# Gavinli-lgf/belief-planning

Hardware: AMD Instinct MI355X
Metric: branch-MPC solves/sec (whole node), highway N=20 M=3 branches, batch 4096 egos (higher is better)
Workload: dtype f64; 1 GPU; highway BranchMPC_CVaR closed loop, N=20, NB=1, m=3 (T=64, U=61), 4096 egos per GPU; batch_per_gpu=4096, global_batch=4096, world_size=1, parallelism=ego-sharded dp1, loop=per step: k_env + solve launches

## Files before the change

### __graft_entry__.py

```python
import os
import sys

REPO = os.path.dirname(os.path.abspath(__file__))
PKG = os.path.join(REPO, "belief-planning_amd")
for _p in (REPO, PKG, os.path.join(REPO, "tests")):
    if _p not in sys.path:
        sys.path.insert(0, _p)


def build() -> None:
    from bmpc import _lib
    _lib.build(force=True, verbose=True)
    _lib.load()
    import hostsim_lib
    hostsim_lib.build()
    import bmpc.plan
    import MPC_branch
    import highway_branch_dyn
    print("build ok:", _lib.SO_PATH)


def smoke() -> None:
    import numpy as np
    from bmpc import plan
    from bmpc.scenarios import highway_desc, highway_policy_rows, seeded_batch
    from oracle.ecos_ipm import ecos_solve
    from oracle.model import HighwayModel, highway_policies
    from oracle.tree import CVaRController

    B = 4
    x, z, xref, tgt = seeded_batch(B, seed=0)
    pl = plan.BatchPlan(highway_desc(N=10, NB=1), B)
    pl.set_policies(highway_policy_rows(tgt))
    r = pl.solve(x, z, xref)
    assert np.all(r["status"] >= 0), r["status"]
    mdl = HighwayModel(10, 0.1, highway_policies(0.1, tgt[0]))
    Fx = np.array([[0., 1, 0, 0], [0, -1, 0, 0], [0, 0, 0, 1], [0, 0, 0, -1]])
    c = CVaRController(mdl, 10, 1, np.diag([0., 3, 3, 10]), np.diag([1., 100]), Fx,
                       [4 * 3.6 - 1.25, -1.25, .25, .25], np.kron(np.eye(2), [1, -1]).T,
                       [6., 6., .3, .3], [0, 300], xref[0], 0.9, solver=ecos_solve)
    c.solve(x[0], z[0], xref[0])
    J_ref = c.last_info["x"][-1]
    assert abs(r["J"][0] - J_ref) <= 1e-6 * max(1.0, abs(J_ref)), (r["J"][0], J_ref)
    assert np.max(np.abs(r["upred"][0, 0] - c.uPred[0])) <= 1e-4
    import scipy.sparse as sp
    from oracle.qp_ipm import osqp_like_solve
# ... 18 lines not shown
```

### belief-planning_amd/bmpc/_lib.py

```python
from __future__ import annotations

import ctypes as C
import os
import subprocess

PKG_DIR = os.path.dirname(os.path.dirname(os.path.abspath(__file__)))
REPO = os.path.dirname(PKG_DIR)
CSRC = os.path.join(PKG_DIR, "csrc")
INCLUDE = os.path.join(REPO, "include")
SO_PATH = os.path.join(PKG_DIR, "libbmpc.so")
PROF_SO_PATH = os.path.join(PKG_DIR, "libbmpc_prof.so")
HIPCC = os.environ.get("HIPCC", "/opt/rocm/bin/hipcc")
EXTRA_FLAGS = []
ARCH = os.environ.get("BMPC_OFFLOAD_ARCH", "gfx950")


class BmpcUnavailable(RuntimeError):
    """libbmpc.so (the MI355X kernels) cannot be loaded or has no usable HIP device."""


EXPERIMENTAL = os.path.join(CSRC, "experimental")


def _phased() -> bool:
# ... 21 lines not shown

def build(force: bool = False, verbose: bool = False, profile: bool = False) -> str:
    out = PROF_SO_PATH if profile else SO_PATH
    stamp = out + ".srchash"
    want = source_hash()
    if not force and os.path.exists(out) and os.path.exists(stamp):
        with open(stamp) as f:
            if f.read().strip() == want:
                return out
    import tempfile
    from concurrent.futures import ThreadPoolExecutor
    flags = [f"--offload-arch={ARCH}", "-O3", "-std=c++17", "-fPIC",
             "-Wno-unused-value", "-Wno-unused-result", "-Wno-pass-failed",
             *(["-DBMPC_PROFILE"] if profile else []), *EXTRA_FLAGS, "-I" + INCLUDE, "-I" + CSRC,
             *(["-I" + EXPERIMENTAL] if _phased() else [])]
    with tempfile.TemporaryDirectory(prefix="bmpc_build_") as tmp:
        objs = [os.path.join(tmp, os.path.basename(src) + ".o") for src in sources()]
        cmds = [[HIPCC, *flags, "-c", src, "-o", obj] for src, obj in zip(sources(), objs)]
        if verbose:
            for c in cmds:
                print(" ".join(c))
        jobs = int(os.environ.get("MAX_JOBS", "0")) or min(len(cmds), os.cpu_count() or 1)
        with ThreadPoolExecutor(jobs) as pool:
            for f in [pool.submit(subprocess.check_call, c) for c in cmds]:
                f.result()
        link = [HIPCC, f"--offload-arch={ARCH}", "-shared", "-fPIC", *objs, "-o", out + ".tmp"]
        if verbose:
            print(" ".join(link))
        subprocess.check_call(link)
    os.replace(out + ".tmp", out)
    with open(stamp, "w") as f:
        f.write(want + "\n")
    return out


_LIB = None

_SIGS = {
    "bmpc_last_error": (C.c_char_p, []),
    "bmpc_abi_version": (C.c_int, []),
    "bmpc_open": (C.c_int, [C.c_int, C.c_void_p]),
    "bmpc_close": (C.c_int, [C.c_void_p]),
    "bmpc_plan_create": (C.c_int, [C.c_void_p, C.c_void_p, C.c_int, C.c_void_p]),
    "bmpc_plan_destroy": (C.c_int, [C.c_void_p]),
    "bmpc_plan_info": (C.c_int, [C.c_void_p, C.c_void_p]),
    "bmpc_set_policies": (C.c_int, [C.c_void_p, C.c_void_p, C.c_void_p]),
    "bmpc_reset": (C.c_int, [C.c_void_p, C.c_void_p]),
    "bmpc_get_policies": (C.c_int, [C.c_void_p, C.c_void_p]),
    "bmpc_solve": (C.c_int, [C.c_void_p] + [C.c_void_p] * 9),
    "bmpc_solve_device": (C.c_int, [C.c_void_p] + [C.c_void_p] * 10),
    "bmpc_get_tree": (C.c_int, [C.c_void_p] + [C.c_void_p] * 6),
    "bmpc_get_warm_start": (C.c_int, [C.c_void_p] * 4),
    "bmpc_get_counters": (C.c_int, [C.c_void_p] * 2),
    "bmpc_set_warm_start": (C.c_int, [C.c_void_p] * 5),
    "bmpc_get_robust_warm_start": (C.c_int, [C.c_void_p] * 4),
    "bmpc_set_robust_warm_start": (C.c_int, [C.c_void_p] * 5),
    "bmpc_set_transform": (C.c_int, [C.c_void_p] * 5),
    "bmpc_set_fx": (C.c_int, [C.c_void_p] * 3),
    "bmpc_get_transform": (C.c_int, [C.c_void_p] * 4),
    "bmpc_get_branch_dp": (C.c_int, [C.c_void_p] * 2),
    "bmpc_enable_timing": (C.c_int, [C.c_void_p, C.c_int]),
    "bmpc_timing": (C.c_int, [C.c_void_p, C.c_void_p, C.c_void_p]),
    "bmpc_model_eval": (C.c_int, [C.c_void_p, C.c_void_p, C.c_void_p, C.c_int] + [C.c_void_p] * 12),
    "bmpc_model_eval_ref": (C.c_int, [C.c_void_p, C.c_void_p, C.c_void_p, C.c_int, C.c_void_p, C.c_void_p, C.c_int]
                            + [C.c_void_p] * 12),
    "bmpc_set_lane_ref": (C.c_int, [C.c_void_p, C.c_int, C.c_void_p, C.c_void_p]),
# ... 84 lines not shown
```

### belief-planning_amd/csrc/bmpc_core.h

```cpp
#pragma once

#include <stddef.h>
#include <stdint.h>

#include "bmpc.h"

#ifndef BMPC_PHASE_NOCSR
#define BMPC_PHASE_NOCSR 1
#endif
#if BMPC_PHASE_NOCSR && defined(__HIP_DEVICE_COMPILE__)
#define BMPC_FN_CALLS __attribute__((not_tail_called))
#else
#define BMPC_FN_CALLS
#endif
#if defined(__HIPCC__)
#include <hip/hip_runtime.h>
#define BMPC_HD __host__ __device__ __forceinline__
#if defined(BMPC_INLINE_ALL)
#define BMPC_FN __host__ __device__ __forceinline__
#else
#define BMPC_FN __host__ __device__ __attribute__((noinline)) BMPC_FN_CALLS
#endif
#else
#define BMPC_HD inline
#define BMPC_FN inline
#endif

#include <math.h>

namespace bmpc {

#if defined(__HIP_DEVICE_COMPILE__)
#if defined(BMPC_FLAT_SLAB)
#define BMPC_AS_GLOBAL
#else
#define BMPC_AS_GLOBAL __attribute__((address_space(1)))
#endif
#define BMPC_AS_LDS __attribute__((address_space(3)))
#define BMPC_AS_CONST __attribute__((address_space(4)))
#else
#define BMPC_AS_GLOBAL
#define BMPC_AS_LDS
#define BMPC_AS_CONST
#endif
typedef BMPC_AS_GLOBAL double gdouble;
typedef BMPC_AS_LDS double ldouble;
typedef const BMPC_AS_GLOBAL int32_t gint;
// ... 17 lines not shown
#define BMPC_TOPO_COUNT_(n) +1
enum { BMPC_TOPO_N = 0 BMPC_TOPO_FIELDS(BMPC_TOPO_COUNT_) };
#define BMPC_TOPO_MEMBER_(n) IP n;
template <class IP>
struct TopoT {
  BMPC_TOPO_FIELDS(BMPC_TOPO_MEMBER_)
};
typedef const BMPC_AS_LDS int32_t lint;
typedef TopoT<gint*> Topo;
typedef TopoT<lint*> TopoL;

enum { XF_S = 0, XF_BX = BMPC_MAX_N * BMPC_MAX_N, XF_SON = XF_BX + BMPC_MAX_FX, XF_BXSET = XF_SON + 1,
       XF_FX = XF_BXSET + 1, XF_FXSET = XF_FX + BMPC_MAX_FX * BMPC_MAX_N, XF_ROWS = XF_FXSET + 1,
       XF_BROWS = XF_ROWS + BMPC_MAX_FX * BMPC_MAX_N, XF_ROWSET = XF_BROWS + BMPC_MAX_FX,
       XF_COUNT = XF_ROWSET + 1 };

enum { ECO_FX = 0, ECO_W1 = BMPC_MAX_FX * BMPC_MAX_N, ECO_QQ = ECO_W1 + BMPC_MAX_N * BMPC_MAX_N,
       ECO_BX = ECO_QQ + BMPC_MAX_N * BMPC_MAX_N, ECO_COUNT = ECO_BX + BMPC_MAX_FX };

struct Plan {
  bmpc_plan_desc desc;
  int n, d, N, NB, m, nFx, nFu, Nc;
  int Ncol, zNB;
  int T, U, nbranch, bdim, ncones, nlevels;
  int oX, oU, oRho, oSig, oMup, oMum, oS, oJ, nv;
  int neq;
  int rFx, rFu, rRisk, rPos, nlp, nrows;
  int ng;
  int nsm;
  int lds_M, lds_piv, lds_rhs, lds_rhs2, lds_red, nlds;
  int lds_w, lds_wu, lds_fx, lds_fu, nconst;
  int nlds_lean;
  int lds_scr, nscr;
  int cgrp;
  int maxq;
  double W1[BMPC_MAX_N * BMPC_MAX_N];
  double Wu[BMPC_MAX_D * BMPC_MAX_D];
  double QQ[BMPC_MAX_N * BMPC_MAX_N];
  double RR[BMPC_MAX_D * BMPC_MAX_D];
  Topo t;
  int toff[BMPC_TOPO_N];
  int ntab;
  const double* lref;
  int nlref;
};

template <class X>
BMPC_HD double fxv(const BMPC_AS_CONST Plan& P, const X& ex, int r, int j) {
  if constexpr (X::kTransform) return ex.eco[ECO_FX + r * P.n + j];
  else return ex.lds[P.lds_fx + r * P.n + j];
}
template <class X>
BMPC_HD double fuv(const BMPC_AS_CONST Plan& P, const X& ex, int r, int j) {
  return ex.lds[P.lds_fu + r * P.d + j];
}
template <class X>
BMPC_HD double w1v(const BMPC_AS_CONST Plan& P, const X& ex, int r, int j) {
  if constexpr (X::kTransform) return ex.eco[ECO_W1 + r * P.n + j];
  else return P.W1[r * P.n + j];
}
template <class X>
BMPC_HD double qqv(const BMPC_AS_CONST Plan& P, const X& ex, int i, int j) {
  if constexpr (X::kTransform) return ex.eco[ECO_QQ + i * P.n + j];
  else return P.QQ[i * P.n + j];
}
template <class X>
// ... 324 lines not shown
```

### belief-planning_amd/csrc/bmpc_dev.h

```cpp
#pragma once

#include <hip/hip_runtime.h>

#include <type_traits>

#include "bmpc_env_merge.h"
#include "bmpc_env_quad.h"
#include "bmpc_hmm.h"
#include "bmpc_plan.h"
#include "bmpc_qp.h"
#include "bmpc_qpplan.h"
#include "bmpc_record.h"
#include "bmpc_solve.h"

namespace bmpc {
namespace dev {

#ifndef BMPC_WPE
#define BMPC_WPE 4
#endif


#ifndef BMPC_DPP_REDUCE
#define BMPC_DPP_REDUCE 1
// ... 2 lines not shown
constexpr bool kDppBlock = BMPC_DPP_REDUCE == 1 || BMPC_DPP_REDUCE == 2;

template <bool TR, bool TL = true>
struct DevExecT {
  static constexpr bool kTransform = TR;
  static constexpr bool kCoupLds = TL;
  using tab_ptr = typename std::conditional<TL, lint*, gint*>::type;
  int lane;
  ldouble* lds;
  tab_ptr tab;
  ldouble* eco;
  static constexpr int nlanes = 64;
  static constexpr bool kBqpWave = true;
  static constexpr bool kInlineG = true;
  static constexpr bool kRowLanes = true;
  __device__ double rlane(double v, int l) const {
    return __hiloint2double(__builtin_amdgcn_readlane(__double2hiint(v), l),
                            __builtin_amdgcn_readlane(__double2loint(v), l));
  }
  static constexpr int kTaskLanes = 4;
  static constexpr int kConeRegRows = 8;
  __device__ double tsum(double v) const {
    v += dpp_d<0xB1>(v);
    v += dpp_d<0x4E>(v);
    return v;
  }
  template <int S>
  __device__ double tget(double v) const { return dpp_d<S | (S << 2) | (S << 4) | (S << 6)>(v); }
  __device__ double gsum(double v, int g) const { return group_reduce<0, kDppWave>(v, g); }
  __device__ double gmax(double v, int g) const { return group_reduce<1, kDppWave>(v, g); }
  __device__ double gmin(double v, int g) const { return group_reduce<2, kDppWave>(v, g); }
  __device__ void sync() const { __syncthreads(); }
  __device__ bool uniform(bool b) const { return __builtin_amdgcn_readfirstlane((int)b) != 0; }
  __device__ double sum(double v) const { return wave_reduce<0, kDppWave>(v); }
  __device__ double max(double v) const { return wave_reduce<1, kDppWave>(v); }
  __device__ double min(double v) const { return wave_reduce<2, kDppWave>(v); }
  template <int K>
  __device__ void sum_n(double* v) const {
#pragma unroll
    for (int k = 0; k < K; ++k) v[k] = sum(v[k]);
  }
  template <int K>
  __device__ void min_n(double* v) const {
#pragma unroll
    for (int k = 0; k < K; ++k) v[k] = min(v[k]);
  }
};

using DevExec = DevExecT<false>;

#ifndef BMPC_BLK_RED2
#define BMPC_BLK_RED2 1
#endif
template <bool TR, bool TL, int NW>
struct DevBlockExecT {
  static constexpr bool kTransform = TR;
  static constexpr bool kCoupLds = TL;
  using tab_ptr = typename std::conditional<TL, lint*, gint*>::type;
  int lane;
  ldouble* lds;
  tab_ptr tab;
  ldouble* eco;
  ldouble* red;
  static constexpr int nlanes = 64 * NW;
  static constexpr int kBatchDiv = NW;
  static constexpr bool kRowLanes = true;
  static constexpr int kTaskLanes = 4;
  static constexpr int kConeRegRows = NW == 4 ? 4 : 8;
  static constexpr int kConeBatch = NW == 4 ? 2 : 4;
  static constexpr int kRedMax = 16;
  __device__ double tsum(double v) const {
    v += dpp_d<0xB1>(v);
    v += dpp_d<0x4E>(v);
    return v;
  }
  template <int S>
  __device__ double tget(double v) const { return dpp_d<S | (S << 2) | (S << 4) | (S << 6)>(v); }
  __device__ double gsum(double v, int g) const { return group_reduce<0, kDppBlock>(v, g); }
  __device__ double gmax(double v, int g) const { return group_reduce<1, kDppBlock>(v, g); }
  __device__ double gmin(double v, int g) const { return group_reduce<2, kDppBlock>(v, g); }
  __device__ void sync() const { __syncthreads(); }
  __device__ bool uniform(bool b) const { return __builtin_amdgcn_readfirstlane((int)b) != 0; }
  template <int OP, int K>
  __device__ void reduce(double* v) const {
    static_assert(K <= kRedMax, "reduction scratch");
#pragma unroll
    for (int k = 0; k < K; ++k) v[k] = wave_reduce<OP, kDppBlock>(v[k]);
    const int wv = lane >> 6;
#if BMPC_BLK_RED2
    ldouble* turn = red + 2 * kRedMax * NW + wv;
    const int odd = __builtin_amdgcn_readfirstlane((int)*turn);
    ldouble* buf = red + (odd ? kRedMax * NW : 0);
    if ((lane & 63) == 0) {
#pragma unroll
      for (int k = 0; k < K; ++k) buf[k * NW + wv] = v[k];
      *turn = odd ? 0.0 : 1.0;
    }
#else
    ldouble* buf = red;
    __syncthreads();
    if ((lane & 63) == 0)
#pragma unroll
      for (int k = 0; k < K; ++k) red[k * NW + wv] = v[k];
// ... 515 lines not shown
```

### belief-planning_amd/csrc/bmpc_ipm.h

```cpp
#pragma once

#include <type_traits>

#include "bmpc_tree.h"
#include "bmpc_wave.h"

#ifndef BMPC_EQUIL
#define BMPC_EQUIL 1
#endif
#ifndef BMPC_EQUIL_ITERS
#define BMPC_EQUIL_ITERS 3
#endif
#ifndef BMPC_TS_POST_RB_MIN
#define BMPC_TS_POST_RB_MIN 8
#endif
#ifndef BMPC_TS_POST_RB
#define BMPC_TS_POST_RB 4
#endif
#ifndef BMPC_PAIR_REFINE
#define BMPC_PAIR_REFINE 1
#endif
#ifndef BMPC_BLK_WAVE_SUBST
#define BMPC_BLK_WAVE_SUBST 1
#endif
// ... 3455 lines not shown
            const int b = t.cone_b[k], ii = t.cone_i[k];
            on = col == P.oSig + b || col == P.oMup + b + ii || col == P.oMum + b + ii ||
                 (t.br_child0[c] >= 0 && col == P.oRho + c);
          } else {
            on = col == P.oJ || col == P.oRho;
          }
          if (on) m = fmax(m, 1.0 / (ge[t.cone_off[k]] * cf));
        }
        if (col < P.oMup) {
          const int b = col < P.oSig ? col - P.oRho : col - P.oSig;
          m = fmax(m, 1.0 / (ae[T * NX + b] * cf));
        } else if (col >= P.oMum && col < P.oS) {
          const int j = col - P.oMum;
          m = fmax(m, fabs(p[j] / P.desc.ralpha) / (ae[T * NX + j / P.m] * cf));
        }
      }
      cm[col] = m;
    }
    ex.sync();
    auto fac = [](double v) { return fabs(v) < 1e-6 ? 1.0 : sqrt(v); };
    for (int i = ex.lane; i < nv; i += ex.nlanes) xe[i] *= fac(cm[i]);
    for (int i = ex.lane; i < neq; i += ex.nlanes) ae[i] *= fac(am[i]);
    for (int i = ex.lane; i < nr; i += ex.nlanes) ge[i] *= fac(gm[i]);
    ex.sync();
  }
}

struct IpmResult {
  int exit_flag;
  int iters;
  double pcost;
};

template <class X, int NX, int NU>
BMPC_HD IpmResult ipm_solve(const X ex, const Ctx& C) {
  CPlan& P = *C.P;
  CLayout& L = *C.L;
  gdouble* ws = C.ws;
  const int nv = P.nv, neq = P.neq, nr = P.nrows;
  gdouble* x = ws + L.x;
  gdouble* y = ws + L.y;
  gdouble* z = ws + L.z;
  gdouble* s = ws + L.s;
  gdouble* lam = ws + L.lam;
  gdouble* x1 = ws + L.x1;
  gdouble* y1 = ws + L.y1;
  gdouble* z1 = ws + L.z1;
  gdouble* x2 = ws + L.x2;
  gdouble* y2 = ws + L.y2;
  gdouble* z2 = ws + L.z2;
  gdouble* dz = ws + L.dz;
  gdouble* ds = ws + L.ds;
  gdouble* rx = ws + L.rx;
  gdouble* ry = ws + L.ry;
  gdouble* rz = ws + L.rz;
  gdouble* hv = ws + L.hvec;
  gdouble* bv = ws + L.bvec;
  gdouble* tA = ws + L.ta;
  gdouble* tA2 = ws + L.ta2;
  gdouble* ya = ws + L.ya;
  gdouble* ra = ws + L.ra;
  gdouble* rb = ws + L.rb;
  gdouble* rc = ws + L.rc;
  const double feastol = P.desc.feastol, abstol = P.desc.abstol, reltol = P.desc.reltol;
  const double deg = (double)(P.nlp + P.ncones);
  IpmResult res{EXIT_MAXIT, 0, 0.0};
  BMPC_PROF(ws, L, PROF_TOTAL);
  BMPC_TIC(t_init);
// ... 262 lines not shown
#else
        lane_batch<8>(ex, 0, nv, [&](int i) { return x[i] + (alpha * x2[i]); }, [&](int i, double v) { x[i] = v; });
        lane_batch(ex, 0, neq, [&](int i) { return y[i] + (alpha * y2[i]); }, [&](int i, double v) { y[i] = v; });
#endif
        struct ZS { double z, s; };
        lane_batch<4>(ex, 0, nr, [&](int i) { return ZS{z[i] + alpha * z2[i], s[i] + alpha * rc[i]}; },
                   [&](int i, ZS v) { z[i] = v.z; s[i] = v.s; });
        tau += alpha * dtau;
        kap += alpha * dkap;
        ex.sync();
      }
    }
    if (!ok) {
      BMPC_TRACE("   backtrack (it %d) to the best iterate (it %d, score %.3e)\n", it, best_it, best_score);
      if (best_score < 1e300 && (ws[L.misc + MISC_BEST] != best_score || ws[L.misc + MISC_BEST + 1] != best_tau)) {
        res.exit_flag = EXIT_GUARD;
        res.iters = it;
        return res;
      }
      const bool inacc = bs_ok_cx && bs_pres < 1e-4 && bs_dres < 1e-4 &&
                         (bs_gap < 5e-5 || (bs_relgap >= 0.0 && bs_relgap < 5e-5));
      lane_batch<16>(ex, 0, nv, [&](int i) { return ws[L.bestx + i] / best_tau; }, [&](int i, double v) { ws[L.sol + i] = v; });
      ex.sync();
      res.exit_flag = inacc ? EXIT_OPTIMAL + EXIT_INACC : EXIT_NUMERICS;
      res.iters = it;
      res.pcost = bs_pcost;
      (void)best_it;
      return res;
    }
  }
  return res;
}

}
```

### belief-planning_amd/csrc/bmpc_plan.cpp

```cpp
#include <stdlib.h>
#include "bmpc_plan.h"

#include <algorithm>

#include <math.h>
#include <string.h>

#include <deque>

namespace bmpc {

namespace {

void sqrtm_sym(const double* A, int n, double* out) {
  double a[BMPC_MAX_N][BMPC_MAX_N], v[BMPC_MAX_N][BMPC_MAX_N];
  for (int i = 0; i < n; ++i)
    for (int j = 0; j < n; ++j) {
      a[i][j] = A[i * n + j];
      v[i][j] = i == j ? 1.0 : 0.0;
    }
  for (int sweep = 0; sweep < 100; ++sweep) {
    double off = 0.0;
    for (int i = 0; i < n; ++i)
      for (int j = i + 1; j < n; ++j) off += a[i][j] * a[i][j];
// ... 245 lines not shown
  hp.cone_c.push_back(-1);
  hp.cone_q.push_back(2 + d);
  hp.cone_off.push_back(row);
  hp.u_cone[0] = k;
  row += 2 + d;
  P.nrows = row;
  P.maxq = 0;
  for (int q : hp.cone_q) P.maxq = q > P.maxq ? q : P.maxq;
  while (P.cgrp < 64 && P.maxq > 8 * P.cgrp) P.cgrp <<= 1;
  if (desc.controller != BMPC_CTRL_CVAR) {
    P.oS = T * n + U * d;
    P.oRho = P.oSig = P.oMup = P.oMum = P.oS;
    P.oJ = P.oS + T * P.Nc;
    P.ncones = 0;
    P.nv = P.oJ;
    P.neq = T * n;
    P.rFx = 0;
    P.rFu = T * P.Nc;
    P.rRisk = P.rFu + U * P.nFu;
    P.rPos = P.rRisk;
    P.nlp = P.rPos + T * P.Nc;
    P.nrows = P.nlp;
    P.ng = 0;
    P.nsm = 0;
  }
  const int ncoup = P.nsm * P.nsm + 3 * P.nsm;
  P.lds_red = 0;
  P.lds_w = 0;
  P.lds_wu = P.lds_w + n * n;
  P.lds_fx = P.lds_wu + d * d;
  P.lds_fu = P.lds_fx + P.nFx * n;
  P.nconst = P.lds_fu + P.nFu * d;
  P.lds_scr = std::max(64, (P.nconst + 7) & ~7);
  P.nscr = desc.controller == BMPC_CTRL_CVAR && P.lds_scr + ncoup + T * P.Nc <= 1248 ? T * P.Nc : 0;
  P.lds_piv = P.lds_scr + P.nscr;
  P.lds_rhs = P.lds_piv + P.nsm;
  P.lds_rhs2 = P.lds_rhs + P.nsm;
  P.lds_M = P.lds_rhs2 + P.nsm;
  P.nlds = P.lds_M + P.nsm * P.nsm;
  P.nlds_lean = P.lds_M;
  if (P.nscr > 0 && P.nlds > 1248) return "internal: the tree-solve LDS staging overflows the 16-egos-per-CU budget";

  double Qm[BMPC_MAX_N * BMPC_MAX_N], Rm[BMPC_MAX_D * BMPC_MAX_D];
  for (int i = 0; i < n * n; ++i) Qm[i] = desc.Q[i];
  for (int i = 0; i < d * d; ++i) Rm[i] = desc.R[i];
  weight_root(Qm, n, P.W1);
  weight_root(Rm, d, P.Wu);
  for (int i = 0; i < n; ++i)
    for (int j = 0; j < n; ++j) {
      double s = 0.0;
      for (int r = 0; r < n; ++r) s += P.W1[r * n + i] * P.W1[r * n + j];
      P.QQ[i * n + j] = s;
    }
  for (int i = 0; i < d; ++i)
    for (int j = 0; j < d; ++j) {
      double s = 0.0;
      for (int r = 0; r < d; ++r) s += P.Wu[r * d + i] * P.Wu[r * d + j];
      P.RR[i * d + j] = s;
    }

#define BMPC_TOPO_HOSTVEC_(n) &hp.n,
  std::vector<int32_t>* tabs[] = {BMPC_TOPO_FIELDS(BMPC_TOPO_HOSTVEC_)};
#undef BMPC_TOPO_HOSTVEC_
  hp.blob.clear();
  hp.blob_off.clear();
  for (auto* v : tabs) {
    hp.blob_off.push_back(hp.blob.size());
    hp.blob.insert(hp.blob.end(), v->begin(), v->end());
// ... 125 lines not shown
```

Before: 80590 solves/s.

## Keep IPM iteration scalars in LDS to cut register pressure

Adds a record-based IPM solve path that stores the per-iteration scalar state (tau, kappa, best-iterate stats, step quantities) in a small LDS area and reloads it uniformly via readfirstlane, instead of holding it in registers across the whole loop. The layout pointer is hidden behind an opaque SGPR asm so the compiler re-derives offsets and does not keep them live. The aim is to lower VGPR/SGPR pressure and spilling in the large solver kernel, at the cost of extra LDS traffic and a slightly changed LDS plan layout. A compile flag and a rec0 variant build allow comparison with the old register-local path.

```diff
diff --git a/__graft_entry__.py b/__graft_entry__.py
--- a/__graft_entry__.py
+++ b/__graft_entry__.py
@@ -12,6 +12,7 @@
     from bmpc import _lib
     _lib.build(force=True, verbose=True)
     _lib.load()
+    _lib.build_variant("rec0", ["-DBMPC_ITER_RECORD=0"])
     import hostsim_lib
     hostsim_lib.build()
     import bmpc.plan
diff --git a/belief-planning_amd/bmpc/_lib.py b/belief-planning_amd/bmpc/_lib.py
--- a/belief-planning_amd/bmpc/_lib.py
+++ b/belief-planning_amd/bmpc/_lib.py
@@ -77,6 +77,16 @@
     with open(stamp, "w") as f:
         f.write(want + "\n")
     return out
+
+
+def build_variant(tag: str, flags, force: bool = False) -> str:
+    global SO_PATH
+    keep_path, keep_flags = SO_PATH, EXTRA_FLAGS[:]
+    SO_PATH, EXTRA_FLAGS[:] = os.path.join(PKG_DIR, f"libbmpc_{tag}.so"), list(flags)
+    try:
+        return build(force=force)
+    finally:
+        SO_PATH, EXTRA_FLAGS[:] = keep_path, keep_flags
 
 
 _LIB = None
diff --git a/belief-planning_amd/csrc/bmpc_core.h b/belief-planning_amd/csrc/bmpc_core.h
--- a/belief-planning_amd/csrc/bmpc_core.h
+++ b/belief-planning_amd/csrc/bmpc_core.h
@@ -13,6 +13,10 @@
 #else
 #define BMPC_FN_CALLS
 #endif
+#ifndef BMPC_ITER_RECORD
+#define BMPC_ITER_RECORD 1
+#endif
+#define BMPC_ITER_LDS 32
 #if defined(__HIPCC__)
 #include <hip/hip_runtime.h>
 #define BMPC_HD __host__ __device__ __forceinline__
@@ -96,6 +100,7 @@
   int lds_w, lds_wu, lds_fx, lds_fu, nconst;
   int nlds_lean;
   int lds_scr, nscr;
+  int lds_it;
   int cgrp;
   int maxq;
   double W1[BMPC_MAX_N * BMPC_MAX_N];
diff --git a/belief-planning_amd/csrc/bmpc_dev.h b/belief-planning_amd/csrc/bmpc_dev.h
--- a/belief-planning_amd/csrc/bmpc_dev.h
+++ b/belief-planning_amd/csrc/bmpc_dev.h
@@ -58,6 +58,11 @@
   __device__ double gmin(double v, int g) const { return group_reduce<2, kDppWave>(v, g); }
   __device__ void sync() const { __syncthreads(); }
   __device__ bool uniform(bool b) const { return __builtin_amdgcn_readfirstlane((int)b) != 0; }
+  __device__ double uniform(double v) const {
+    return __hiloint2double(__builtin_amdgcn_readfirstlane(__double2hiint(v)),
+                            __builtin_amdgcn_readfirstlane(__double2loint(v)));
+  }
+  static constexpr bool kIterLds = BMPC_ITER_RECORD != 0;
   __device__ double sum(double v) const { return wave_reduce<0, kDppWave>(v); }
   __device__ double max(double v) const { return wave_reduce<1, kDppWave>(v); }
   __device__ double min(double v) const { return wave_reduce<2, kDppWave>(v); }
@@ -95,6 +100,7 @@
   static constexpr int kConeRegRows = NW == 4 ? 4 : 8;
   static constexpr int kConeBatch = NW == 4 ? 2 : 4;
   static constexpr int kRedMax = 16;
+  static constexpr bool kIterRecord = false;
   __device__ double tsum(double v) const {
     v += dpp_d<0xB1>(v);
     v += dpp_d<0x4E>(v);
diff --git a/belief-planning_amd/csrc/bmpc_ipm.h b/belief-planning_amd/csrc/bmpc_ipm.h
--- a/belief-planning_amd/csrc/bmpc_ipm.h
+++ b/belief-planning_amd/csrc/bmpc_ipm.h
@@ -3511,8 +3511,484 @@
   double pcost;
 };
 
+enum {
+  IT_TAU = 0, IT_KAP, IT_RESX0, IT_RESY0, IT_RESZ0,
+  IT_BEST, IT_BEST_TAU, IT_BEST_IT,
+  IT_BS_PRES, IT_BS_DRES, IT_BS_RELGAP, IT_BS_GAP, IT_BS_PCOST, IT_BS_OK_CX,
+  IT_RT, IT_MU, IT_KT,
+  IT_DEN, IT_DTAU_A, IT_DKAP_A, IT_SIGMA, IT_ETA1, IT_SMU, IT_DTAU, IT_DKAP,
+  IT_COUNT
+};
+static_assert(IT_COUNT <= BMPC_ITER_LDS, "the iteration record's LDS area (bmpc_core.h)");
+template <class X, class = void>
+struct iter_lds { static constexpr bool value = false; };
+template <class X>
+struct iter_lds<X, decltype((void)X::kIterLds)> { static constexpr bool value = X::kIterLds; };
+
+template <class T>
+BMPC_HD T* opaque_ptr(T* p) {
+#if defined(__HIP_DEVICE_COMPILE__)
+  p = uniform_ptr(p);
+  asm volatile("" : "+s"(p));
+#endif
+  return p;
+}
+
+template <class X>
+BMPC_HD double ex_uniform(const X& ex, double v) {
+  if constexpr (iter_lds<X>::value) return ex.uniform(v);
+  else return v;
+}
+
+template <class X, bool LDS = iter_lds<X>::value>
+struct IterRec {
+  double v[IT_COUNT];
+  BMPC_HD IterRec(const X&, CPlan&) {}
+  BMPC_HD double ld(int k) const { return v[k]; }
+  BMPC_HD void st(int k, double a) { v[k] = a; }
+};
+template <class X>
+struct IterRec<X, true> {
+  const X& ex;
+  volatile ldouble* p;
+  BMPC_HD IterRec(const X& e, CPlan& P) : ex(e), p(e.lds + P.lds_it) {}
+  BMPC_HD double ld(int k) const { return ex.uniform((double)p[k]); }
+  BMPC_HD void st(int k, double a) { p[k] = a; }
+};
+
+#if BMPC_ITER_RECORD
 template <class X, int NX, int NU>
-BMPC_HD IpmResult ipm_solve(const X ex, const Ctx& C) {
+BMPC_HD IpmResult ipm_solve_record(const X ex, const Ctx& C) {
+  CPlan& P = *C.P;
+  CLayout& L = *C.L;
+  gdouble* ws = C.ws;
+  const int nv = P.nv, neq = P.neq, nr = P.nrows;
+  IterRec<X> R(ex, P);
+  auto LL = [&]() -> CLayout& { return *(iter_lds<X>::value ? opaque_ptr(C.L) : C.L); };
+  IpmResult res{EXIT_MAXIT, 0, 0.0};
+  BMPC_PROF(ws, L, PROF_TOTAL);
+  BMPC_TIC(t_init);
+  if (BMPC_EQUIL) equilibrate<X, NX, NU>(ex, C);
+  build_hb<X, NX, NU>(ex, C, ws + L.hvec, ws + L.bvec);
+  identity_scaling(ex, C);
+  if (!kkt_factor<X, NX, NU>(ex, C, true) || !kkt_coupling<X, NX, NU>(ex, C, 0)) {
+    res.exit_flag = EXIT_NUMERICS;
+    return res;
+  }
+  {
+    gdouble* tA = ws + L.ta;
+    lane_batch<16>(ex, 0, nv, [&](int i) { return 0.0; }, [&](int i, double v) { tA[i] = v; });
+    ex.sync();
+  }
+  kkt_solve_flat<X, NX, NU>(ex, C, ws + L.ta, ws + L.bvec, ws + L.hvec, ws + L.x, ws + L.y2, ws + L.z2,
+                            BMPC_NITREF_INIT);
+  {
+    const gdouble* gq = ws + L.geq;
+    const gdouble* z2 = ws + L.z2;
+    gdouble* ra = ws + L.ra;
+    lane_batch<16>(ex, 0, nr, [&](int i) { return -(BMPC_EQUIL ? gq[i] : 1.0) * z2[i]; }, [&](int i, double v) { ra[i] = v; });
+    ex.sync();
+  }
+  bring2cone(ex, C, ws + L.ra, ws + L.s);
+  if (BMPC_EQUIL) {
+    const gdouble* gq = ws + L.geq;
+    gdouble* s = ws + L.s;
+    lane_batch<16>(ex, 0, nr, [&](int i) { return gq[i] * s[i]; }, [&](int i, double v) { s[i] = v; });
+    ex.sync();
+  }
+  {
+    gdouble* ej = BMPC_IPM_LEAN_PASSES ? ws + L.ej : ws + L.ta;
+    gdouble* ya = ws + L.ya;
+    gdouble* ra = ws + L.ra;
+    lane_batch<16>(ex, 0, nv, [&](int i) { return i == P.oJ ? -1.0 : 0.0; }, [&](int i, double v) { ej[i] = v; });
+    lane_batch(ex, 0, neq, [&](int i) { return 0.0; }, [&](int i, double v) { ya[i] = v; });
+    lane_batch<16>(ex, 0, nr, [&](int i) { return 0.0; }, [&](int i, double v) { ra[i] = v; });
+    ex.sync();
+    kkt_solve_flat<X, NX, NU>(ex, C, ej, ya, ra, ws + L.x2, ws + L.y, ws + L.z2, BMPC_NITREF_INIT);
+  }
+  if (BMPC_EQUIL) {
+    const gdouble* gq = ws + L.geq;
+    gdouble* z2 = ws + L.z2;
+    lane_batch<16>(ex, 0, nr, [&](int i) { return gq[i] * z2[i]; }, [&](int i, double v) { z2[i] = v; });
+    ex.sync();
+  }
+  bring2cone(ex, C, ws + L.z2, ws + L.z);
+  if (BMPC_EQUIL) {
+    const gdouble* gq = ws + L.geq;
+    gdouble* z = ws + L.z;
+    lane_batch<16>(ex, 0, nr, [&](int i) { return z[i] / gq[i]; }, [&](int i, double v) { z[i] = v; });
+    ex.sync();
+  }
+  R.st(IT_TAU, 1.0);
+  R.st(IT_KAP, 1.0);
+  R.st(IT_RESX0, BMPC_EQUIL ? fmax(1.0, 1.0 / ws[L.xeq + P.oJ]) : 1.0);
+  {
+    const gdouble* bv = ws + L.bvec;
+    const gdouble* aq = ws + L.aeq;
+    R.st(IT_RESY0, fmax(1.0, sqrt(lane_sum(ex, 0, neq, [&](int i) {
+      const double v = BMPC_EQUIL ? bv[i] / aq[i] : bv[i];
+      return v * v;
+    }))));
+  }
+  {
+    const gdouble* hv = ws + L.hvec;
+    const gdouble* gq = ws + L.geq;
+    R.st(IT_RESZ0, fmax(1.0, sqrt(lane_sum(ex, 0, nr, [&](int i) {
+      const double v = BMPC_EQUIL ? hv[i] / gq[i] : hv[i];
+      return v * v;
+    }))));
+  }
+  R.st(IT_BEST, 1e300);
+  R.st(IT_BEST_TAU, 1.0);
+  R.st(IT_BEST_IT, 0.0);
+  BMPC_TOC(ws, L, PROF_INIT, t_init);
+  R.st(IT_BS_PRES, 0.0), R.st(IT_BS_DRES, 0.0), R.st(IT_BS_RELGAP, 0.0), R.st(IT_BS_GAP, 0.0), R.st(IT_BS_PCOST, 0.0);
+  R.st(IT_BS_OK_CX, 0.0);
+
+  for (int it = 0; it <= P.desc.maxit; ++it) {
+#if defined(BMPC_PROFILE) && defined(__HIP_DEVICE_COMPILE__)
+    {
+      BMPC_TIC(t_lat);
+      const double probe = *(volatile const gdouble*)(ws + LL().bestx + ex.lane);
+      if (probe == 1.2345e300) ws[LL().prof + PROF_STEP] += 0.0;
+      BMPC_TOC(ws, L, PROF_STEP, t_lat);
+    }
+#endif
+    BMPC_TIC(t_res);
+    apply_AT<X, NX, NU>(ex, C, ws + LL().y, ws + LL().rx);
+    apply_GT<X, NX, NU>(ex, C, ws + LL().z, ws + LL().ta);
+    double acx[2] = {0.0, 0.0}, acy[3] = {0.0, 0.0, 0.0}, acz[5] = {0.0, 0.0, 0.0, 0.0, 0.0};
+    {
+      const gdouble* x = ws + LL().x;
+      const gdouble* xq = ws + LL().xeq;
+      const gdouble* tA = ws + LL().ta;
+      gdouble* rx = ws + LL().rx;
+      gdouble* tA2 = ws + LL().ta2;
+      const double tau = R.ld(IT_TAU);
+      struct R2b { double v, rs, xs; };
+      lane_batch<8>(ex, 0, nv, [&](int i) {
+        const double xi = x[i], q = BMPC_EQUIL ? xq[i] : 1.0;
+        const double v = rx[i] + (tA[i] + (i == P.oJ ? tau : 0.0));
+        return R2b{v, v / q, q * xi};
+      }, [&](int i, R2b r) {
+        rx[i] = r.v;
+        if (BMPC_IPM_LEAN_PASSES) tA2[i] = -r.v;
+        acx[0] += r.rs * r.rs;
+        acx[1] += r.xs * r.xs;
+      });
+    }
+    apply_A<X, NX, NU>(ex, C, ws + LL().x, ws + LL().ry);
+    {
+      const gdouble* y = ws + LL().y;
+      const gdouble* bv = ws + LL().bvec;
+      const gdouble* aq = ws + LL().aeq;
+      gdouble* ry = ws + LL().ry;
+      const double tau = R.ld(IT_TAU);
+      struct R4 { double v, rs, a, ys; };
+      lane_batch<8>(ex, 0, neq, [&](int i) {
+        const double yi = y[i], bi = bv[i], q = BMPC_EQUIL ? aq[i] : 1.0;
+        const double v = bi * tau - ry[i];
+        return R4{v, v / q, bi * yi, q * yi};
+      }, [&](int i, R4 r) { ry[i] = r.v; acy[0] += r.rs * r.rs; acy[1] += r.a; acy[2] += r.ys * r.ys; });
+    }
+    apply_G<X, NX, NU>(ex, C, ws + LL().x, ws + LL().rz);
+    {
+      const gdouble* z = ws + LL().z;
+      const gdouble* s = ws + LL().s;
+      const gdouble* hv = ws + LL().hvec;
+      const gdouble* gq = ws + LL().geq;
+      gdouble* rz = ws + LL().rz;
+      const double tau = R.ld(IT_TAU);
+      struct R7 { double v, rs, a, zs, ss, sz; };
+      lane_batch<4>(ex, 0, nr, [&](int i) {
+        const double zi = z[i], si = s[i], hi = hv[i], q = BMPC_EQUIL ? gq[i] : 1.0;
+        const double v = hi * tau - rz[i] - si;
+        return R7{v, v / q, hi * zi, q * zi, si / q, si * zi};
+      }, [&](int i, R7 r) { rz[i] = r.v; acz[0] += r.rs * r.rs; acz[1] += r.a; acz[2] += r.zs * r.zs; acz[3] += r.ss * r.ss; acz[4] += r.sz; });
+    }
+    ex.sync();
+    double rsum[10] = {acy[1], acz[1], acx[1], acy[2], acz[2], acz[3], acz[4], acy[0], acz[0], acx[0]};
+    ex.template sum_n<10>(rsum);
+    const double tau = R.ld(IT_TAU), kap = R.ld(IT_KAP);
+    const double cx = ws[LL().x + P.oJ];
+    const double by = rsum[0], hz = rsum[1];
+    const double rt = kap + cx + by + hz;
+    const double nx = sqrt(rsum[2]), ny = sqrt(rsum[3]);
+    const double nz = sqrt(rsum[4]), ns = sqrt(rsum[5]);
+    const double sz = rsum[6];
+    const double kt = kap * tau;
+    const double mu = (sz + kt) / ((double)(P.nlp + P.ncones) + 1.0);
+    R.st(IT_RT, rt);
+    R.st(IT_MU, mu);
+    R.st(IT_KT, kt);
+    const double gap = sz / (tau * tau);
+    const double pcost = cx / tau, dcost = -(hz + by) / tau;
+    double relgap = -1.0;
+    if (pcost < 0.0) relgap = gap / (-pcost);
+    else if (dcost > 0.0) relgap = gap / dcost;
+    const double nry = neq ? sqrt(rsum[7]) / fmax(R.ld(IT_RESY0) + nx, 1.0) : 0.0;
+    const double nrz = sqrt(rsum[8]) / fmax(R.ld(IT_RESZ0) + nx + ns, 1.0);
+    const double pres = fmax(nry, nrz) / tau;
+    const double dres = sqrt(rsum[9]) / fmax(R.ld(IT_RESX0) + ny + nz, 1.0) / tau;
+    BMPC_TOC(ws, L, PROF_RESID, t_res);
+    const double reltol = P.desc.reltol;
+    double pinfres = -1.0, dinfres = -1.0;
+    if ((hz + by) / fmax(ny + nz, 1.0) < -reltol) {
+      const gdouble* rx = ws + LL().rx;
+      const gdouble* xq = ws + LL().xeq;
+      gdouble* ra = ws + LL().ra;
+      lane_batch<16>(ex, 0, nv, [&](int i) { return (rx[i] - (i == P.oJ ? tau : 0.0)) / (BMPC_EQUIL ? xq[i] : 1.0); },
+                     [&](int i, double v) { ra[i] = v; });
+      ex.sync();
+      pinfres = sqrt(vdot(ex, ra, ra, nv)) / fmax(ny + nz, 1.0);
+    }
+    if (cx / fmax(nx, 1.0) < -reltol) {
+      const gdouble* rb = ws + LL().rb;
+      const gdouble* aq = ws + LL().aeq;
+      const gdouble* gq = ws + LL().geq;
+      const gdouble* s = ws + LL().s;
+      gdouble* ra = ws + LL().ra;
+      apply_A<X, NX, NU>(ex, C, ws + LL().x, ws + LL().rb);
+      const double a1 = sqrt(lane_sum(ex, 0, neq, [&](int i) {
+        const double v = rb[i] / (BMPC_EQUIL ? aq[i] : 1.0);
+        return v * v;
+      })) / fmax(nx, 1.0);
+      apply_G<X, NX, NU>(ex, C, ws + LL().x, ra);
+      lane_batch<16>(ex, 0, nr, [&](int i) { return (ra[i] + s[i]) / (BMPC_EQUIL ? gq[i] : 1.0); },
+                     [&](int i, double v) { ra[i] = v; });
+      ex.sync();
+      const double a2 = sqrt(vdot(ex, ra, ra, nr)) / fmax(nx + ns, 1.0);
+      dinfres = fmax(a1, a2);
+    }
+    auto check = [&](double ft, double at, double rtl) -> int {
+      if (!(tau > 0.0 && kap >= 0.0)) return 99;
+      if ((-cx > 0.0 || -by - hz >= -at) && pres < ft && dres < ft &&
+          (gap < at || (relgap >= 0.0 && relgap < rtl)))
+        return EXIT_OPTIMAL;
+      if (dinfres >= 0.0 && dinfres < ft && tau < kap) return EXIT_DINF;
+      if ((pinfres >= 0.0 && pinfres < ft && tau < kap) ||
+          (tau < ft && kap < ft && pinfres >= 0.0 && pinfres < ft))
+        return EXIT_PINF;
+      return 99;
+    };
+    const double score = fmax(fmax(pres, dres), relgap >= 0.0 ? relgap : 1e300);
+    if (score < R.ld(IT_BEST)) {
+      R.st(IT_BEST, score);
+      R.st(IT_BEST_IT, (double)it);
+      R.st(IT_BEST_TAU, tau);
+      R.st(IT_BS_PRES, pres), R.st(IT_BS_DRES, dres), R.st(IT_BS_RELGAP, relgap), R.st(IT_BS_GAP, gap), R.st(IT_BS_PCOST, pcost);
+      R.st(IT_BS_OK_CX, (-cx > 0.0 || -by - hz >= -5e-5) ? 1.0 : 0.0);
+      if (ex.lane == 0) {
+        ws[LL().misc + MISC_BEST] = score;
+        ws[LL().misc + MISC_BEST + 1] = tau;
+      }
+      const gdouble* x = ws + LL().x;
+      lane_batch<16>(ex, 0, nv, [&](int i) { return x[i]; }, [&](int i, double v) { ws[LL().bestx + i] = v; });
+      ex.sync();
+    }
+    BMPC_TRACE("it %3d pcost %+.16e dcost %+.16e gap %.16e pres %.16e dres %.16e kap %.16e tau %.16e"
+               " nx %.16e ny %.16e nz %.16e ns %.16e best %.3e\n",
+               it, pcost, dcost, gap, pres, dres, kap, tau, nx, ny, nz, ns, R.ld(IT_BEST));
+    int code = check(P.desc.feastol, P.desc.abstol, reltol);
+    if (code == 99 && it == P.desc.maxit) {
+      const int c2 = check(1e-4, 5e-5, 5e-5);
+      code = c2 == 99 ? EXIT_MAXIT : c2 + EXIT_INACC;
+    }
+    if (code != 99) BMPC_TRACE("   code %d (it %d)\n", code, it);
+    if (code != 99) {
+      const gdouble* x = ws + LL().x;
+      lane_batch<16>(ex, 0, nv, [&](int i) { return x[i] / tau; }, [&](int i, double v) { ws[LL().sol + i] = v; });
+      ex.sync();
+      res.exit_flag = code;
+      res.iters = it;
+      res.pcost = pcost;
+      return res;
+    }
+    const int nref = ex.uniform(score < BMPC_REFSCORE2) ? BMPC_NITREF2 : ex.uniform(score < BMPC_REFSCORE) ? BMPC_NITREF : 0;
+    bool ok = ex.uniform(compute_scaling(ex, C, ws + LL().s, ws + LL().z));
+    if (ok) ok = ex.uniform(kkt_factor<X, NX, NU>(ex, C, false));
+    if (ok) {
+      gdouble* ej = BMPC_IPM_LEAN_PASSES ? ws + LL().ej : ws + LL().ta;
+#if !BMPC_IPM_LEAN_PASSES
+      {
+        const gdouble* rx = ws + LL().rx;
+        gdouble* tA2 = ws + LL().ta2;
+        lane_batch<16>(ex, 0, nv, [&](int i) { return i == P.oJ ? -1.0 : 0.0; }, [&](int i, double v) { ej[i] = v; });
+        lane_batch<16>(ex, 0, nv, [&](int i) { return -rx[i]; }, [&](int i, double v) { tA2[i] = v; });
+      }
+#endif
+      apply_W(ex, C, 0, ws + LL().lam, ws + LL().rb, 1.0, ws + LL().rz, 1.0);
+#if BMPC_FLAT_PAIR
+      kkt_pair_rhs<X, NX, NU>(ex, C, ej, ws + LL().ta2, ws + LL().rb);
+      ok = ex.uniform(kkt_coupling<X, NX, NU>(ex, C, 2));
+      if (ok) {
+        kkt_pair_back<X, NX, NU>(ex, C, nref == 0);
+        if (nref > 0) {
+#if BMPC_PAIR_REFINE
+          kkt_refine_pair<X, NX, NU>(ex, C, ej, ws + LL().bvec, ws + LL().k_t3, ws + LL().x1, ws + LL().y1, ws + LL().z1, ws + LL().ta2,
+                                     ws + LL().ry, ws + LL().k_t3b, ws + LL().x2, ws + LL().y2, ws + LL().z2, nref);
+#else
+          kkt_refine<X, NX, NU>(ex, C, ej, ws + LL().bvec, ws + LL().k_t3, ws + LL().x1, ws + LL().y1, ws + LL().z1, nref);
+          kkt_refine<X, NX, NU>(ex, C, ws + LL().ta2, ws + LL().ry, ws + LL().k_t3b, ws + LL().x2, ws + LL().y2, ws + LL().z2, nref);
+#endif
+        }
+      }
+#else
+      ok = ex.uniform(kkt_solve_pair<X, NX, NU>(ex, C, ej, ws + LL().ta2, ws + LL().rb, nref));
+#endif
+    }
+    if (ok) {
+#if BMPC_IPM_LEAN_PASSES
+      double by1, by2;
+      dot2_pair(ex, ws + LL().bvec, ws + LL().y1, ws + LL().y2, neq, ws + LL().hvec, ws + LL().z1, ws + LL().z2, nr, by1, by2);
+#else
+      const double by1 = dot2(ex, ws + LL().bvec, ws + LL().y1, neq, ws + LL().hvec, ws + LL().z1, nr),
+                   by2 = dot2(ex, ws + LL().bvec, ws + LL().y2, neq, ws + LL().hvec, ws + LL().z2, nr);
+#endif
+      {
+        const double tau = R.ld(IT_TAU), kap = R.ld(IT_KAP);
+        const double den = kap / tau - (ws[LL().x1 + P.oJ] + by1);
+        const double dk_aff = -R.ld(IT_KT);
+        const double dtau_a = (R.ld(IT_RT) + dk_aff / tau + ws[LL().x2 + P.oJ] + by2) / den;
+        R.st(IT_DEN, den);
+        R.st(IT_DTAU_A, dtau_a);
+        R.st(IT_DKAP_A, (dk_aff - kap * dtau_a) / tau);
+      }
+      const LpSteps lpa = affine_dirs(ex, C, ws + LL().z2, ws + LL().z1, R.ld(IT_DTAU_A), ws + LL().lam, ws + LL().rb, ws + LL().ds);
+      double a_aff = max_step2<X, BMPC_IPM_LEAN_PASSES != 0>(ex, C, ws + LL().lam, ws + LL().ds, ws + LL().rb, lpa.a1, lpa.a2);
+      {
+        const double tau = R.ld(IT_TAU), kap = R.ld(IT_KAP);
+        const double dtau_a = R.ld(IT_DTAU_A), dkap_a = R.ld(IT_DKAP_A);
+        if (dtau_a < 0.0) a_aff = fmin(a_aff, -tau / dtau_a);
+        if (dkap_a < 0.0) a_aff = fmin(a_aff, -kap / dkap_a);
+        a_aff = fmax(0.0, fmin(a_aff, 0.999));
+        double sigma = (1.0 - a_aff) * (1.0 - a_aff) * (1.0 - a_aff);
+        sigma = fmin(1.0, fmax(1e-4, sigma));
+        const double eta1 = 1.0 - sigma;
+        const double smu = sigma * R.ld(IT_MU);
+        R.st(IT_SIGMA, sigma);
+        R.st(IT_ETA1, eta1);
+        R.st(IT_SMU, smu);
+        combined_rhs(ex, C, ws + LL().lam, ws + LL().ds, ws + LL().rb, ws + LL().rz, smu, eta1);
+      }
+      {
+        const gdouble* rx = ws + LL().rx;
+        const gdouble* ry = ws + LL().ry;
+        gdouble* tA = ws + LL().ta;
+        gdouble* ya = ws + LL().ya;
+        const double eta1 = R.ld(IT_ETA1);
+        lane_batch<16>(ex, 0, nv, [&](int i) { return -eta1 * rx[i]; }, [&](int i, double v) { tA[i] = v; });
+        lane_batch(ex, 0, neq, [&](int i) { return eta1 * ry[i]; }, [&](int i, double v) { ya[i] = v; });
+        ex.sync();
+      }
+      kkt_solve_flat<X, NX, NU>(ex, C, ws + LL().ta, ws + LL().ya, ws + LL().rb, ws + LL().x2, ws + LL().y2, ws + LL().z2, nref);
+      {
+        const double d2 = dot2(ex, ws + LL().bvec, ws + LL().y2, neq, ws + LL().hvec, ws + LL().z2, nr);
+        const double tau = R.ld(IT_TAU);
+        const double dk_c = -R.ld(IT_KT) - R.ld(IT_DTAU_A) * R.ld(IT_DKAP_A) + R.ld(IT_SMU);
+        const double dtau = (R.ld(IT_ETA1) * R.ld(IT_RT) + dk_c / tau + ws[LL().x2 + P.oJ] + d2) / R.ld(IT_DEN);
+        R.st(IT_DTAU, dtau);
+        R.st(IT_DKAP, (dk_c - R.ld(IT_KAP) * dtau) / tau);
+      }
+      double nonfinite = 0.0;
+#if !BMPC_IPM_LEAN_PASSES
+      {
+        const gdouble* x1 = ws + LL().x1;
+        const gdouble* y1 = ws + LL().y1;
+        gdouble* x2 = ws + LL().x2;
+        gdouble* y2 = ws + LL().y2;
+        const double dtau = R.ld(IT_DTAU);
+        lane_batch<8>(ex, 0, nv, [&](int i) { return x2[i] + (dtau * x1[i]); }, [&](int i, double v) {
+          x2[i] = v;
+          if (!isfinite(v)) nonfinite = 1.0;
+        });
+        lane_batch(ex, 0, neq, [&](int i) { return y2[i] + (dtau * y1[i]); }, [&](int i, double v) { y2[i] = v; });
+        ex.sync();
+      }
+#endif
+      const LpSteps lpc = combined_dirs(ex, C, ws + LL().z2, ws + LL().z1, R.ld(IT_DTAU), ws + LL().ds, ws + LL().rb, ws + LL().rc);
+      double a = max_step2<X, BMPC_IPM_LEAN_PASSES != 0>(ex, C, ws + LL().lam, ws + LL().ds, ws + LL().rb, lpc.a1, lpc.a2);
+      const double dtau = R.ld(IT_DTAU), dkap = R.ld(IT_DKAP);
+      {
+        const double tau = R.ld(IT_TAU), kap = R.ld(IT_KAP);
+        if (dtau < 0.0) a = fmin(a, -tau / dtau);
+        if (dkap < 0.0) a = fmin(a, -kap / dkap);
+      }
+      a = fmin(a, 0.999);
+      const double alpha = ex_uniform(ex, a * 0.99);
+#if BMPC_IPM_LEAN_PASSES
+      ok = ex.uniform(isfinite(dtau) && alpha > 1e-10);
+      if (ok) {
+        const gdouble* x1 = ws + LL().x1;
+        const gdouble* x2 = ws + LL().x2;
+        gdouble* x = ws + LL().x;
+        lane_batch<8>(ex, 0, nv, [&](int i) {
+          const double v = x2[i] + (dtau * x1[i]);
+          if (!isfinite(v)) nonfinite = 1.0;
+          return x[i] + (alpha * v);
+        }, [&](int i, double v) { x[i] = v; });
+        ok = ex.uniform(ex.max(nonfinite) == 0.0);
+      }
+#else
+      const double fin = ex.max(nonfinite);
+      ok = ex.uniform(fin == 0.0 && isfinite(dtau) && alpha > 1e-10);
+#endif
+      BMPC_TRACE("   step den %.16e dtau_a %.16e a_aff %.16e sigma %.16e dtau %.16e alpha %.16e nref %d ok %d\n",
+                 R.ld(IT_DEN), R.ld(IT_DTAU_A), a_aff, R.ld(IT_SIGMA), dtau, alpha, nref, (int)ok);
+      if (ok) {
+        {
+          const gdouble* y1 = ws + LL().y1;
+          const gdouble* y2 = ws + LL().y2;
+          gdouble* y = ws + LL().y;
+#if BMPC_IPM_LEAN_PASSES
+          lane_batch(ex, 0, neq, [&](int i) { return y[i] + (alpha * (y2[i] + (dtau * y1[i]))); },
+                     [&](int i, double v) { y[i] = v; });
+#else
+          const gdouble* x2 = ws + LL().x2;
+          gdouble* x = ws + LL().x;
+          (void)y1;
+          lane_batch<8>(ex, 0, nv, [&](int i) { return x[i] + (alpha * x2[i]); }, [&](int i, double v) { x[i] = v; });
+          lane_batch(ex, 0, neq, [&](int i) { return y[i] + (alpha * y2[i]); }, [&](int i, double v) { y[i] = v; });
+#endif
+        }
+        {
+          const gdouble* z2 = ws + LL().z2;
+          const gdouble* rc = ws + LL().rc;
+          gdouble* z = ws + LL().z;
+          gdouble* s = ws + LL().s;
+          struct ZS { double z, s; };
+          lane_batch<4>(ex, 0, nr, [&](int i) { return ZS{z[i] + alpha * z2[i], s[i] + alpha * rc[i]}; },
+                     [&](int i, ZS v) { z[i] = v.z; s[i] = v.s; });
+        }
+        R.st(IT_TAU, R.ld(IT_TAU) + alpha * dtau);
+        R.st(IT_KAP, R.ld(IT_KAP) + alpha * dkap);
+        ex.sync();
+      }
+    }
+    if (!ok) {
+      const double best_score = R.ld(IT_BEST), best_tau = R.ld(IT_BEST_TAU);
+      BMPC_TRACE("   backtrack (it %d) to the best iterate (it %d, score %.3e)\n", it, (int)R.ld(IT_BEST_IT), best_score);
+      if (best_score < 1e300 && (ws[LL().misc + MISC_BEST] != best_score || ws[LL().misc + MISC_BEST + 1] != best_tau)) {
+        res.exit_flag = EXIT_GUARD;
+        res.iters = it;
+        return res;
+      }
+      const double bs_relgap = R.ld(IT_BS_RELGAP);
+      const bool inacc = R.ld(IT_BS_OK_CX) != 0.0 && R.ld(IT_BS_PRES) < 1e-4 && R.ld(IT_BS_DRES) < 1e-4 &&
+                         (R.ld(IT_BS_GAP) < 5e-5 || (bs_relgap >= 0.0 && bs_relgap < 5e-5));
+      lane_batch<16>(ex, 0, nv, [&](int i) { return ws[LL().bestx + i] / best_tau; }, [&](int i, double v) { ws[LL().sol + i] = v; });
+      ex.sync();
+      res.exit_flag = inacc ? EXIT_OPTIMAL + EXIT_INACC : EXIT_NUMERICS;
+      res.iters = it;
+      res.pcost = R.ld(IT_BS_PCOST);
+      return res;
+    }
+  }
+  return res;
+}
+#endif
+template <class X, int NX, int NU>
+BMPC_HD IpmResult ipm_solve_locals(const X ex, const Ctx& C) {
   CPlan& P = *C.P;
   CLayout& L = *C.L;
   gdouble* ws = C.ws;
@@ -3841,4 +4317,17 @@
   return res;
 }
 
-}
+template <class X, class = void>
+struct iter_record { static constexpr bool value = BMPC_ITER_RECORD != 0; };
+template <class X>
+struct iter_record<X, decltype((void)X::kIterRecord)> { static constexpr bool value = BMPC_ITER_RECORD != 0 && X::kIterRecord; };
+template <class X, int NX, int NU>
+BMPC_HD IpmResult ipm_solve(const X ex, const Ctx& C) {
+#if BMPC_ITER_RECORD
+  if constexpr (iter_record<X>::value) return ipm_solve_record<X, NX, NU>(ex, C);
+  else
+#endif
+    return ipm_solve_locals<X, NX, NU>(ex, C);
+}
+
+}
diff --git a/belief-planning_amd/csrc/bmpc_plan.cpp b/belief-planning_amd/csrc/bmpc_plan.cpp
--- a/belief-planning_amd/csrc/bmpc_plan.cpp
+++ b/belief-planning_amd/csrc/bmpc_plan.cpp
@@ -301,8 +301,11 @@
   P.lds_fu = P.lds_fx + P.nFx * n;
   P.nconst = P.lds_fu + P.nFu * d;
   P.lds_scr = std::max(64, (P.nconst + 7) & ~7);
-  P.nscr = desc.controller == BMPC_CTRL_CVAR && P.lds_scr + ncoup + T * P.Nc <= 1248 ? T * P.Nc : 0;
-  P.lds_piv = P.lds_scr + P.nscr;
+  const bool it_tail = P.lds_scr - P.nconst >= BMPC_ITER_LDS;
+  const int nit = desc.controller == BMPC_CTRL_CVAR && !it_tail ? BMPC_ITER_LDS : 0;
+  P.nscr = desc.controller == BMPC_CTRL_CVAR && P.lds_scr + nit + ncoup + T * P.Nc <= 1248 ? T * P.Nc : 0;
+  P.lds_it = it_tail ? P.nconst : P.lds_scr + P.nscr;
+  P.lds_piv = P.lds_scr + P.nscr + nit;
   P.lds_rhs = P.lds_piv + P.nsm;
   P.lds_rhs2 = P.lds_rhs + P.nsm;
   P.lds_M = P.lds_rhs2 + P.nsm;
```

Result: faster. 82540 solves/s, median of 6 (+2.4%).
